# darcamo/pyphysim

Hardware: AMD Instinct MI355X
Metric: Monte Carlo realizations/sec (whole node) + SER abs-error vs ref (higher is better)
Workload: dtype f64

## Files before the change

include/mcle.h:

```cpp
#ifndef MCLE_H
#define MCLE_H

#include <stddef.h>
#include <stdint.h>

#ifdef __cplusplus
extern "C" {
#endif

#define MCLE_VERSION 1

enum { MCLE_OK = 0, MCLE_E_INVAL = -1, MCLE_E_HIP = -2, MCLE_E_NOMEM = -3, MCLE_E_STATE = -4,
       MCLE_E_UNSUPPORTED = -5  };
enum { MCLE_F32 = 0, MCLE_F64 = 1 };
enum { MCLE_DEMOD_MINDIST = 0, MCLE_DEMOD_QAM_SLICER = 1 };
enum { MCLE_CONST_GENERIC = 0, MCLE_CONST_QAM = 1, MCLE_CONST_BPSK = 2 };

typedef struct mcle_ctx mcle_ctx;

typedef struct mcle_counters {
    uint64_t n_realizations;
    uint64_t n_skipped;
    uint64_t sym_errors;
    uint64_t sym_errors_sq;
// ... 10 lines not shown
int mcle_ctx_destroy(mcle_ctx* ctx);
int mcle_ctx_set_stream(mcle_ctx* ctx, void* hip_stream);
int mcle_ctx_get_stream(mcle_ctx* ctx, void** hip_stream);
int mcle_ctx_sync(mcle_ctx* ctx);
int mcle_ctx_trim_scratch(mcle_ctx* ctx);
int mcle_ctx_device_info(mcle_ctx* ctx, int* n_cu, int* lds_bytes, char* name, int name_len);
int mcle_ctx_last_kernel(mcle_ctx* ctx, char* name, int len);
int mcle_malloc(mcle_ctx* ctx, size_t bytes, void** d_ptr);
int mcle_free(mcle_ctx* ctx, void* d_ptr);
int mcle_memset(mcle_ctx* ctx, void* d_ptr, int value, size_t bytes);
int mcle_memcpy_h2d(mcle_ctx* ctx, void* d_dst, const void* src, size_t bytes);
int mcle_memcpy_d2h(mcle_ctx* ctx, void* dst, const void* d_src, size_t bytes);
int mcle_memcpy_2d(mcle_ctx* ctx, void* d_dst, size_t dst_pitch, const void* d_src, size_t src_pitch,
                   size_t row_bytes, size_t rows);
enum {
    MCLE_OPT_NO_MFMA = 0,
    MCLE_OPT_MFMA_VARIANT = 1,
    MCLE_OPT_GRID_OVERSUB = 2,
    MCLE_OPT_FLAT_WGS_PER_CU = 3,
    MCLE_OPT_SINGLE_TDL = 4,
    MCLE_OPT_TDL_MFMA_WAVES = 5,
    MCLE_OPT_JAKES_DIRECT = 6,
    MCLE_OPT_F64_GENERIC = 7,
    MCLE_OPT_F64_THREADS = 8,
    MCLE_OPT_BD_RUNTIME_SOLVE = 9,
    MCLE_OPT_DEMOD_NOCERT = 10,
    MCLE_OPT_F64_VARIANT = 11,
    MCLE_OPT_F32_MFMA = 12,
    MCLE_OPT_TDL_KERNEL = 13,
    MCLE_OPT_MIMO_TDL_KERNEL = 14,
    MCLE_OPT_WALK_LEGACY = 15,
    MCLE_OPT_STAGED_GENERIC = 16,
    MCLE_OPT_CODEBOOK_NO_PACK = 17,
    MCLE_OPT_COUNT = 18
};
int mcle_ctx_set_option(mcle_ctx* ctx, int option, long long value);
int mcle_ctx_get_option(mcle_ctx* ctx, int option, long long* value);

int mcle_timer_start(mcle_ctx* ctx);
int mcle_timer_stop_ms(mcle_ctx* ctx, float* ms);

enum { MCLE_HBM_COPY = 0, MCLE_HBM_READ = 1, MCLE_HBM_TRIAD = 2, MCLE_HBM_WRITE = 3,
       MCLE_HBM_NONTEMPORAL = 4 , MCLE_HBM_UNROLL8 = 8  };
int mcle_hbm_stream_rate(mcle_ctx* ctx, int kind, size_t bytes, int reps, int blocks_per_cu, double* gbps);

int mcle_comm_load(const char* rccl_path);
int mcle_comm_unique_id(void* id_out, size_t bytes);
int mcle_comm_init(mcle_ctx* ctx, const void* unique_id, int rank, int world);
int mcle_comm_destroy(mcle_ctx* ctx);
int mcle_comm_info(mcle_ctx* ctx, int* rank, int* world);
int mcle_counters_allreduce(mcle_ctx* ctx, mcle_counters* d_counters, int n);
int mcle_allreduce_f64(mcle_ctx* ctx, double* d_values, size_t n);


int mcle_set_constellation(mcle_ctx* ctx, const double* re_im, int M, int kind);

int mcle_build_demod_grid(const double* re_im, int M, int* G, double* x0, double* y0, double* h,
                          unsigned long long* cells);

int mcle_modulate(mcle_ctx* ctx, int dtype, const int32_t* d_idx, void* d_out, size_t n);
int mcle_demodulate(mcle_ctx* ctx, int dtype, int method, const void* d_rx, int32_t* d_idx,
                    size_t n);
int mcle_count_errors(mcle_ctx* ctx, const int32_t* d_tx_idx, const int32_t* d_rx_idx,
                      size_t n_per_real, size_t n_real, int bits_per_symbol,
                      mcle_counters* d_counters, uint32_t* d_sym_err, uint32_t* d_bit_err);
int mcle_demod_count(mcle_ctx* ctx, int dtype, int method, const void* d_rx,
                     const int32_t* d_tx_idx, size_t n_per_real, size_t n_real,
// ... 429 lines not shown
```

pyphysim_amd/_lib.py:

```python
import ctypes
import importlib.util
import os
from ctypes import (POINTER, Structure, byref, c_char_p, c_double, c_float, c_int, c_int32, c_longlong, c_size_t,
                    c_uint32, c_uint64, c_void_p)

import numpy as np

MCLE_F32, MCLE_F64 = 0, 1
DEMOD_MINDIST, DEMOD_QAM_SLICER = 0, 1
CONST_GENERIC, CONST_QAM, CONST_BPSK = 0, 1, 2
MAX_TAPS = 24
STREAM_DATA, STREAM_NOISE, STREAM_CHAN, STREAM_PHASE, STREAM_PILOT = 0, 1, 2, 3, 4
OPTIONS = {"no_mfma": 0, "mfma_variant": 1, "grid_oversub": 2, "flat_wgs_per_cu": 3, "single_tdl": 4,
           "tdl_mfma_waves": 5, "jakes_direct": 6, "f64_generic": 7,
           "f64_threads": 8, "bd_runtime_solve": 9, "demod_nocert": 10, "f64_variant": 11, "f32_mfma": 12, "tdl_kernel": 13,
           "mimo_tdl_kernel": 14, "walk_legacy": 15, "staged_generic": 16, "codebook_no_pack": 17}

LIB_DIR = os.path.join(os.path.dirname(os.path.abspath(__file__)), "csrc")
LIB_PATH = os.environ.get("MCLE_LIBRARY") or os.path.join(LIB_DIR, "libmcle.so")


class McleError(RuntimeError):
    """Any failure reported by libmcle (message from mcle_last_error)."""


class McleUnsupported(McleError):
    """A valid request outside a fused kernel's envelope (MCLE_E_UNSUPPORTED): use the staged operators."""


class Counters(Structure):
    _fields_ = [(n, c_uint64) for n in ("n_realizations", "n_skipped", "sym_errors", "sym_errors_sq",
                                        "bit_errors", "bit_errors_sq", "n_symbols", "n_bits")]

    def as_dict(self):
        return {n: int(getattr(self, n)) for n, _ in self._fields_}


COUNTER_FIELDS = [n for n, _ in Counters._fields_]


class AwgnCfg(Structure):
    _fields_ = [("n_symbols", c_int32), ("demod_method", c_int32), ("noise_var", c_double)]


class FlatCfg(Structure):
    _fields_ = [("n_symbols", c_int32), ("demod_method", c_int32), ("noise_var", c_double),
                ("Fd", c_double), ("Ts", c_double), ("L", c_int32), ("rayleigh_iid", c_int32)]


# ... 353 lines not shown
```

pyphysim_amd/csrc/c4_select.hpp:

```cpp
#pragma once
#include <cstdio>
#include "../../include/mcle.h"

namespace mcle {

enum : int { WDEC_GENERIC = 0, WDEC_SLICER = 1, WDEC_QAM_CERT = 2, WDEC_QUAD_CERT = 3, WDEC_AXIS4_CERT = 4 };

enum : int {
    C4_THR_DEFAULT = 0,
    C4_THR_R4_AH4 = 256,
    C4_THR_R16_ALT = 257,
    C4_THR_R16_TABLE = 258,
    C4_THR_R16_FUSED = 259,
    C4_THR_WAVE = 260,
    C4_THR_PLANAR = 261,
    C4_THR_WAVE_ALT = 262,
    C4_THR_PW4 = 263,
    C4_THR_PW4_W2 = 264,
    C4_THR_PW_TIME = 265,
    C4_THR_PW_CLASS = 266,
    C4_THR_PW_PLANES = 267,
    C4_THR_PW_HALVES = 268,
    C4_THR_512 = 512,
    C4_THR_1024 = 1024,
};
constexpr bool c4_threads_accepted(long long v) {
    return v == C4_THR_DEFAULT || (v >= C4_THR_R4_AH4 && v <= C4_THR_PW_HALVES) || v == C4_THR_512 || v == C4_THR_1024;
}

struct C4Query {
    bool f64;
    int fft_size, nt, nr, num_used, cp_size;
    int M;
    int dec;
    long long f64_threads, f64_generic, no_mfma, f32_mfma, mfma_variant;
#ifdef MCLE_EXPERIMENTS
    long long f64_variant;
#endif
};

enum : int { C4_REFUSED_SHAPE = 0, C4_GENERIC, C4_PLANAR, C4_FW, C4_QW, C4_PW, C4_MFMA };

struct C4Plan {
    int family = C4_REFUSED_SHAPE;
    bool f64 = true;
    int n = 0, nt = 0, nr = 0;
    int ah = 0;
    int wps = 0;
    int variant = 0;
    bool td = false, rows = false, halves = false;
    char asked = 0;
    int abl = 0;
};

#ifndef MCLE_PLANAR_F32_WPS_PLUS
#define MCLE_PLANAR_F32_WPS_PLUS 2
#endif
#ifndef MCLE_PLANAR_F64_256_WPS3
#define MCLE_PLANAR_F64_256_WPS3 0
#endif
constexpr int planar_wps(bool f64, int n, int nt, int nr, int w64) {
    if (!f64 && w64 <= 3 && ((n == 256 && !(nt == 4 && nr == 4)) || (n == 512 && nr == 2))) return w64 + MCLE_PLANAR_F32_WPS_PLUS;
    if (MCLE_PLANAR_F64_256_WPS3 && f64 && n == 256 && nr <= 3 && w64 == 2) return 3;
    return w64;
}

constexpr int planar_r4_ah(int nr) { return nr == 3 ? 3 : 2; }
constexpr int planar_r4_wps(bool f64, int n, int nt, int nr) {
    const int w64 = nr == 3 ? 2 : nr == 2 ? (n == 256 ? 2 : n == 2048 ? 4 : 3) : (n <= 512 ? 3 : 4);
    return planar_wps(f64, n, nt, nr, w64);
}

#ifdef MCLE_EXPERIMENTS
constexpr bool c4_abl_wave(long long v) { return (v >= 32 && v <= 1024 && (v & (v - 1)) == 0) || v == 2016; }
constexpr bool c4_abl_qw(long long v) { return c4_abl_wave(v) || v == 384; }
constexpr bool c4_abl_planar(long long v) { return c4_abl_qw(v) || v == 1920; }
#endif

inline bool c4_select_planar(const C4Query& q, C4Plan& p) {
    const int n = q.fft_size, nt = q.nt, nr = q.nr;
    const long long thr = q.f64_threads;
    if (!(n == 256 || n == 512 || n == 1024 || n == 2048) || nr < 2 || nr > 4 || nt < 1 || nt > nr) return false;
    if (n == 256 && nt == 2 && nr == 2) return false;
    p.family = C4_PLANAR;
    p.ah = planar_r4_ah(nr);
    p.wps = planar_r4_wps(q.f64, n, nt, nr);
    p.variant = 0;
    if (n == 1024 && nr == 4) {
        const int r16_wps = q.f64 ? 2 : 4, r16_var = q.f64 ? 12 : 4;
        if (nt < 4) {
            if (thr == C4_THR_DEFAULT) p.ah = 4, p.wps = r16_wps, p.variant = r16_var;
            return true;
        }
#ifdef MCLE_EXPERIMENTS
        if (q.f64 && q.f64_variant >= 1 && q.f64_variant <= 3) {
            p.variant = (int)q.f64_variant;
            return true;
        }
        if (q.f64 && c4_abl_planar(q.f64_variant)) {
            p.ah = 4, p.wps = 2, p.variant = 12 | (int)q.f64_variant;
            return true;
        }
#endif
        if (thr == C4_THR_512) return true;
// ... 12 lines not shown
inline C4Plan c4_select(const C4Query& q) {
    const int n = q.fft_size, nt = q.nt, nr = q.nr;
    const long long thr = q.f64_threads;
    const bool sq4 = nt == 4 && nr == 4;
    C4Plan p;
    p.f64 = q.f64, p.n = n, p.nt = nt, p.nr = nr;
    if (!q.f64 && q.f32_mfma && !q.no_mfma && n == 1024 && sq4) {
        p.family = C4_MFMA;
        p.variant = q.mfma_variant ? (int)q.mfma_variant : 36;
        return p;
    }
    const bool has_generic = nt == nr && (nt == 2 || nt == 4);
    const bool want_generic = has_generic && (q.f64_generic || (!q.f64 && q.no_mfma));
    if (!want_generic) {
        const bool wave = q.num_used == n && (q.cp_size & 1) == 0 && q.M <= 256 && q.dec != WDEC_GENERIC;
        const bool wave_thr = thr == C4_THR_DEFAULT || thr == C4_THR_WAVE || thr == C4_THR_WAVE_ALT;
        if (wave && n == 256 && has_generic && wave_thr) {
            p.family = C4_FW;
            p.wps = (thr == C4_THR_WAVE_ALT) == q.f64 ? 2 : 3;
#ifdef MCLE_EXPERIMENTS
            if (q.f64 && sq4 && c4_abl_wave(q.f64_variant)) p.wps = 3, p.abl = (int)q.f64_variant;
#endif
            return p;
        }
        const bool pw_thr = thr == C4_THR_DEFAULT || (thr >= C4_THR_PW_TIME && thr <= C4_THR_PW_HALVES) ||
                            (n == 1024 ? thr == C4_THR_PW4 || thr == C4_THR_PW4_W2 : thr == C4_THR_WAVE || thr == C4_THR_WAVE_ALT);
        if (wave && q.f64 && sq4 && (n == 512 || n == 1024 || n == 2048) && pw_thr) {
            p.family = C4_PW;
            p.wps = n == 2048 ? 2 : 3;
            p.td = thr == C4_THR_PW_TIME;
            p.rows = !p.td && thr != C4_THR_PW_CLASS;
            p.halves = p.rows && (thr == C4_THR_PW_HALVES || (thr != C4_THR_PW_PLANES && n != 512));
            p.asked = thr == C4_THR_PW_PLANES ? 'x' : thr == C4_THR_PW_HALVES ? 'h' : 0;
            if (n != 2048) {
                if (thr == C4_THR_WAVE_ALT || thr == C4_THR_PW4_W2) p.wps = 2;
#ifdef MCLE_EXPERIMENTS
                if ((thr < C4_THR_PW_CLASS || thr > C4_THR_PW_HALVES) && c4_abl_wave(q.f64_variant))
                    p.wps = 3, p.halves = false, p.abl = (int)q.f64_variant;
#endif
            }
            return p;
        }
        if (wave && q.f64 && sq4 && n == 1024 && wave_thr && (q.dec == WDEC_SLICER || q.dec == WDEC_QAM_CERT || q.dec == WDEC_QUAD_CERT)) {
            p.family = C4_QW;
            p.wps = thr == C4_THR_WAVE_ALT ? 2 : 3;
#ifdef MCLE_EXPERIMENTS
            if (c4_abl_qw(q.f64_variant)) p.wps = 3, p.abl = (int)q.f64_variant;
#endif
            return p;
        }
        if (c4_select_planar(q, p)) return p;
    }
    if (has_generic) p.family = C4_GENERIC;
    return p;
}

inline void c4_plan_tag(const C4Plan& p, char* out, int len) {
    const char* dt = p.f64 ? "f64" : "f32";
    switch (p.family) {
        case C4_GENERIC: std::snprintf(out, (size_t)len, "mimo_ofdm_generic<%d,%d> %s", p.n, p.nt, dt); break;
        case C4_PLANAR: std::snprintf(out, (size_t)len, "mimo_ofdm_planar<%d,%d,%d> %s ah%d w%d v%d", p.n, p.nt, p.nr, dt, p.ah, p.wps, p.variant); break;
        case C4_FW: std::snprintf(out, (size_t)len, "mimo_ofdm_fw<%d> %s w%d", p.nt, dt, p.wps); break;
        case C4_QW: std::snprintf(out, (size_t)len, "mimo_ofdm_qw w%d", p.wps); break;
        case C4_PW:
            std::snprintf(out, (size_t)len, "mimo_ofdm_pw<%d>/%s%s%s", p.n / 256, p.td ? "time" : "freq", p.wps == (p.n == 2048 ? 2 : 3) ? "" : "/w2",
                          !p.td && !p.rows ? "/a" : p.asked == 'x' ? "/x" : p.asked == 'h' ? "/h" : "");
// ... 8 lines not shown
```

pyphysim_amd/csrc/capi.hip:

```cpp
#include <cmath>
#include <cstdarg>

#include "c4_select.hpp"
#include "common.hpp"
#include "modem.hpp"

namespace mcle {

static thread_local char g_err[512] = "";

void set_error(const char* fmt, ...) {
    va_list ap;
    va_start(ap, fmt);
    vsnprintf(g_err, sizeof(g_err), fmt, ap);
    va_end(ap);
}

}

using namespace mcle;

int mcle_ctx::bind() const {
    MCLE_HIP(hipSetDevice(device));
    return MCLE_OK;
// ... 177 lines not shown
}

int mcle_ctx_get_stream(mcle_ctx* ctx, void** hip_stream) {
    MCLE_REQUIRE(ctx != nullptr && hip_stream != nullptr, "null argument");
    *hip_stream = (void*)ctx->stream;
    return MCLE_OK;
}

int mcle_ctx_set_option(mcle_ctx* ctx, int option, long long value) {
    MCLE_REQUIRE(ctx != nullptr, "null context");
    MCLE_REQUIRE(option >= 0 && option < MCLE_OPT_COUNT, "unknown option %d", option);
    bool ok = false;
    switch (option) {
        case MCLE_OPT_NO_MFMA: case MCLE_OPT_SINGLE_TDL: case MCLE_OPT_JAKES_DIRECT: case MCLE_OPT_F64_GENERIC: case MCLE_OPT_BD_RUNTIME_SOLVE: case MCLE_OPT_DEMOD_NOCERT: case MCLE_OPT_F32_MFMA: case MCLE_OPT_WALK_LEGACY: case MCLE_OPT_STAGED_GENERIC: case MCLE_OPT_CODEBOOK_NO_PACK: ok = value == 0 || value == 1; break;
        case MCLE_OPT_TDL_KERNEL: ok = value >= 0 && value <= 4; break;
#ifdef MCLE_EXPERIMENTS
        case MCLE_OPT_MIMO_TDL_KERNEL: ok = value >= 0 && value <= 255; break;
#else
        case MCLE_OPT_MIMO_TDL_KERNEL: ok = value >= 0 && value <= 2; break;
#endif
#ifdef MCLE_EXPERIMENTS
        case MCLE_OPT_F64_VARIANT: ok = value >= 0 && value <= 2047; break;
#else
        case MCLE_OPT_F64_VARIANT:
            MCLE_REQUIRE(value == 0, "option MCLE_OPT_F64_VARIANT: the timing-bound variants are compiled with -DMCLE_EXPERIMENTS only");
            ok = true;
            break;
#endif
        case MCLE_OPT_MFMA_VARIANT: ok = value == 0 || value == 36 || value == 32 || value == 30 || value == 21; break;
        case MCLE_OPT_GRID_OVERSUB: ok = value >= 0 && value <= 64; break;
        case MCLE_OPT_FLAT_WGS_PER_CU: ok = value >= 0 && value <= 4096; break;
        case MCLE_OPT_TDL_MFMA_WAVES: ok = value == 0 || value == 2 || value == 3 || value == 32; break;
        case MCLE_OPT_F64_THREADS: ok = c4_threads_accepted(value); break;
    }
    MCLE_REQUIRE(ok, "option %d: value %lld out of range", option, value);
    ctx->opt[option] = value;
    return MCLE_OK;
}

int mcle_ctx_trim_scratch(mcle_ctx* ctx) {
    MCLE_REQUIRE(ctx != nullptr, "null context");
    MCLE_HIP(hipSetDevice(ctx->device));
    MCLE_HIP(hipStreamSynchronize(ctx->stream));
    if (ctx->d_scratch) MCLE_HIP(hipFree(ctx->d_scratch));
    ctx->d_scratch = nullptr;
    ctx->scratch_bytes = 0;
    return MCLE_OK;
}

int mcle_ctx_get_option(mcle_ctx* ctx, int option, long long* value) {
    MCLE_REQUIRE(ctx != nullptr && value != nullptr, "null argument");
    MCLE_REQUIRE(option >= 0 && option < MCLE_OPT_COUNT, "unknown option %d", option);
    *value = ctx->opt[option];
    return MCLE_OK;
}

int mcle_ctx_sync(mcle_ctx* ctx) {
    MCLE_REQUIRE(ctx != nullptr, "null context");
    MCLE_HIP(hipSetDevice(ctx->device));
    MCLE_HIP(hipStreamSynchronize(ctx->stream));
    return MCLE_OK;
}

int mcle_ctx_device_info(mcle_ctx* ctx, int* n_cu, int* lds_bytes, char* name, int name_len) {
    MCLE_REQUIRE(ctx != nullptr, "null context");
    if (n_cu) *n_cu = ctx->n_cu;
// ... 303 lines not shown
```

pyphysim_amd/csrc/pipeline_mimo_pw.hip:

```cpp
#include "mimo_planar_common.hpp"
#include "walk_f64.hpp"

namespace mcle {

constexpr int kPwPlane = 4 * 272;
__host__ __device__ __forceinline__ int pw_slot(int a, int e) { return a * 272 + e + (e >> 4); }
__host__ __device__ __forceinline__ int pw_mtime(int h, int c) { return (c & 3) * 64 + (c >> 2) * 16 + (h & 3) * 4 + (h >> 2); }
template <int NW> constexpr int pw_lab_stride() { return 16 * NW + 16; }
template <int NW> constexpr size_t pw_static_lds() {
    return (size_t)((kBmLdsDoubles + 1) & ~1) * sizeof(double) + (size_t)64 * pw_lab_stride<NW>() + 2 * (d64_rec<4, 4>() + 1) * sizeof(double2) +
           64 * sizeof(unsigned) + sizeof(WgTotals);
}

__device__ __forceinline__ void pw_row_swap(uint32_t& x, uint32_t& y) {
#if defined(__HIP_DEVICE_COMPILE__)
#if __has_builtin(__builtin_amdgcn_permlane16_swap)
    const auto s = __builtin_amdgcn_permlane16_swap(x, y, false, false);
    x = s[0];
    y = s[1];
#else
    const bool odd = (__lane_id() & 16) != 0;
    const uint32_t give = odd ? x : y, got = (uint32_t)__shfl_xor((int)give, 16);
    if (odd) x = got;
    else y = got;
#endif
#endif
}

template <int NW, int J, bool STUB>
__device__ __forceinline__ void pw_first_stage(const unsigned char* lab_row, const double2* s_txtab, const double2* __restrict__ g_tw,
                                               double2 (&v)[16]) {
    const uint4* lab = reinterpret_cast<const uint4*>(lab_row);
    if constexpr (NW == 4) {
#pragma unroll
        for (int i = 0; i < 4; ++i) {
            const uint4 L = lab[i];
            const uint32_t wds[4] = {L.x, L.y, L.z, L.w};
#pragma unroll
            for (int uu = 0; uu < 4; ++uu) {
                const int u = 4 * i + uu;
                const uint32_t w = wds[uu];
                double2 X0, X1, X2, X3;
                if constexpr (STUB) {
                    X0 = X1 = X2 = X3 = mk<double>((double)w, 1.0);
// ... 60 lines not shown
                else v[u] = cmulc(S, g_tw[16 * J * u]);
            }
        }
    } else {
        static_assert(NW == 2, "first stage");
#pragma unroll
        for (int i = 0; i < 2; ++i) {
            const uint4 L = lab[i];
            const uint32_t wds[4] = {L.x, L.y, L.z, L.w};
#pragma unroll
            for (int uu = 0; uu < 8; ++uu) {
                const int u = 8 * i + uu;
                const uint32_t w = wds[uu >> 1] >> (16 * (uu & 1));
                double2 X0, X1;
                if constexpr (STUB) {
                    X0 = X1 = mk<double>((double)(w & 0xFFFFu), 1.0);
                } else {
                    X0 = s_txtab[w & 0xFFu];
                    X1 = s_txtab[(w >> 8) & 0xFFu];
                }
                const double2 S = J ? csub(X0, X1) : cadd(X0, X1);
                if constexpr (J == 0) v[u] = S;
                else if (u == 0) v[u] = S;
                else v[u] = cmulc(S, g_tw[16 * J * u]);
            }
        }
    }
}

template <int NW, int DEC, int WPS, bool TD = false, int ABL = 0, bool ROWS = !TD, bool XCH = ROWS && !TD>
__global__ __launch_bounds__(64 * NW, WPS) void k_run_mimo_ofdm_pw(MimoParams pp, ModemParams<double> mp, uint64_t seed, uint64_t first,
                                                                   uint64_t count, const double2* __restrict__ g_tw,
                                                                   const double2* __restrict__ g_recs, mcle_counters* counters,
                                                                   uint32_t* __restrict__ sym_out, uint32_t* __restrict__ bit_out) {
    using T = double;
    constexpr int N = 256 * NW, NT = 4, NR = 4, kRec = d64_rec<NT, NR>(), TB = 64 * NW, UU = 16 / NW;
    constexpr int kLabStride = pw_lab_stride<NW>();
    static_assert(NW == 2 || NW == 4 || NW == 8, "wavefronts per realization");
    static_assert(!(TD && ROWS), "the time-domain form keeps the map wavefront = class");
    static_assert(!XCH || (ROWS && ABL == 0), "the exchange in complex halves belongs to the default form by lane row");
    constexpr bool kAhead = ROWS && ABL == 0;
#ifdef MCLE_PW_LATE_B5
    constexpr bool kLateB5 = XCH && kAhead;
#else
    constexpr bool kLateB5 = false;
#endif
    constexpr int kLogNW = NW == 2 ? 1 : NW == 4 ? 2 : 3;
    extern __shared__ __attribute__((aligned(16))) char pw_smem[];
    constexpr int kBm = (kBmLdsDoubles + 1) & ~1;
    __shared__ __attribute__((aligned(16))) double s_bm[kBm];
    __shared__ __attribute__((aligned(16))) unsigned char s_lab[64 * kLabStride];
    __shared__ __attribute__((aligned(16))) cx<T> s_rec[2 * (kRec + 1)];
    __shared__ unsigned s_part[64];
    __shared__ WgTotals totals;
    static_assert(sizeof(s_bm) + sizeof(s_lab) + sizeof(s_rec) + sizeof(s_part) + sizeof(totals) == pw_static_lds<NW>(), "launcher's LDS sum");
    T* s_R = reinterpret_cast<T*>(pw_smem);
    cx<T>* s_table = reinterpret_cast<cx<T>*>(s_R + NW * kPwPlane);
    cx<T>* s_txtab = s_table + ((mp.M + 1) & ~1);

    const int tid = threadIdx.x, lane = tid & 63;
    const int j = __builtin_amdgcn_readfirstlane(tid >> 6);
    const int pj = j & 1;
    const int cp = pp.cp;
    const int per_sym = N * NT;
    const uint64_t row = (uint64_t)pp.n_ofdm_sym * (N + cp);
    const T sigma = (T)sqrt(pp.noise_var);
    const T tx_scale = (T)(1.0 / sqrt((double)NT) / sqrt((double)(N + cp)));
    const T tab_scale = TD ? tx_scale : tx_scale * (T)N;
    const uint32_t mask = (uint32_t)(mp.M - 1);
    for (int m = tid; m < mp.M; m += TB) {
        const cx<T> c = mp.g_table[m];
        s_table[m] = c;
        s_txtab[m] = cscale(c, tab_scale);
    }
    if constexpr (ROWS) bm_tables_to_lds_pairs(s_bm, tid, TB);
    else bm_tables_to_lds(s_bm, tid, TB);
    if (tid == 0) wg_zero(totals);

    T* s_mine = s_R + j * kPwPlane;
    uint2* s_words_mine = reinterpret_cast<uint2*>(s_mine);
    using Pass = std::conditional_t<kAhead, uint32_t, uint64_t>;
    Pass it = 0;
    uint64_t rl_prev = 0;
    cx<T> rec_next = mk<T>(0, 0);
    if (tid < kRec && blockIdx.x < count) rec_next = g_recs[(uint64_t)blockIdx.x * kRec + tid];
    unsigned step = 0;
    if constexpr (kAhead) {
        step = gridDim.x;
        asm volatile("" : "+s"(step));
    }
    auto grid_step = [&]() -> unsigned {
        if constexpr (kAhead) return step;
        else return gridDim.x;
    };
    __syncthreads();
    for (uint64_t rl = blockIdx.x; rl < count; rl += grid_step(), ++it) {
        const Rng rng(seed, first + rl);
        const int buf = (int)(it & 1);
        if (tid < kRec) {
            s_rec[buf * (kRec + 1) + tid] = rec_next;
            if (rl + grid_step() < count) rec_next = g_recs[(rl + grid_step()) * kRec + tid];
        }
        const cx<T>* s_H = s_rec + buf * (kRec + 1);
        const cx<T>* s_G = s_H + NT * NR;
        unsigned se = 0, be = 0;
        for (int os = 0; os < pp.n_ofdm_sym; ++os) {
            if constexpr (!kLateB5) {
                if (it > 0 || os > 0) __syncthreads();
            }
            if constexpr (ROWS && !(ABL & 128)) __builtin_amdgcn_s_waitcnt(0xC07F);
            {
                const int t = opaque(tid);
                Words4 dw;
                if constexpr (ABL & 32) dw.w[0] = dw.w[1] = dw.w[2] = dw.w[3] = (uint32_t)t * 0x01010101u;
                else dw = rng.block(STREAM_DATA, (uint32_t)(((uint64_t)os * per_sym) >> 4) + (uint32_t)t);
                const int q = (t >> 6) ^ (NW / 2), u = (t & 63) >> 2;
#pragma unroll
                for (int s = 0; s < 4; ++s) {
                    const uint32_t w = dw.w[s] & (mask * 0x01010101u);
                    const int g = 4 * (t & 3) + s;
                    unsigned char* dst = s_lab + g * kLabStride + NW * u + q;
#pragma unroll
                    for (int a = 0; a < 4; ++a) dst[a * 16 * kLabStride] = (unsigned char)(w >> (8 * a));
                }
            }
            if constexpr (!ROWS) {
                const int ln = opaque(lane);
                const int r = ln >> 4, h = ln & 15;
                const uint64_t i00 = (uint64_t)r * row + (uint64_t)os * (N + cp) + cp + (j & ~1) + 32 * NW * pj + NW * (uint64_t)pw_mtime(h, 0);
                const uint32_t b0 = (uint32_t)(i00 >> 1);
                uint2* w_even = reinterpret_cast<uint2*>(s_R + (j & ~1) * kPwPlane) + (8 * pj) * 64 + ln;
                uint2* w_odd = reinterpret_cast<uint2*>(s_R + (j | 1) * kPwPlane) + (8 * pj) * 64 + ln;
#pragma unroll
                for (int cc = 0; cc < 8; ++cc) {
                    Words4 b;
                    if constexpr (ABL & 128) b.w[0] = b.w[1] = b.w[2] = b.w[3] = b0 + cc;
                    else b = rng.block(STREAM_NOISE, b0 + (uint32_t)(NW / 2) * (uint32_t)pw_mtime(0, cc));
                    w_even[cc * 64] = make_uint2(b.w[0], b.w[1]);
                    w_odd[cc * 64] = make_uint2(b.w[2], b.w[3]);
                }
            }
            auto account_prev = [&]() {
                if (tid == 0 && os == 0 && it > 0) {
                    const unsigned* qq = s_part + (buf ^ 1) * 32;
                    unsigned ts = 0, tb = 0;
#pragma unroll
                    for (int i = 0; i < NW; ++i) {
                        ts += qq[2 * i];
                        tb += qq[2 * i + 1];
                    }
                    uint64_t rp = rl_prev;
                    if constexpr (kAhead) {
                        uint64_t here = rl;
                        asm volatile("" : "+s"(here));
                        rp = here - step;
                    }
                    wg_account(totals, ts, tb, s_rec[(buf ^ 1) * (kRec + 1) + 2 * NT * NR].x != 0.0, rp, sym_out, bit_out);
                }
            };
            if constexpr (!ROWS) {
                __syncthreads();
                account_prev();
            }
            cx<T> v[16];
            if constexpr (TD) {
                const int ln = opaque(lane);
                const unsigned char* lab = s_lab + ln * kLabStride;
                if constexpr (NW == 4) {
                    switch (j) {
                        case 0: pw_first_stage<4, 0, (ABL & 32) != 0>(lab, s_txtab, g_tw, v); break;
                        case 1: pw_first_stage<4, 1, (ABL & 32) != 0>(lab, s_txtab, g_tw, v); break;
                        case 2: pw_first_stage<4, 2, (ABL & 32) != 0>(lab, s_txtab, g_tw, v); break;
                        default: pw_first_stage<4, 3, (ABL & 32) != 0>(lab, s_txtab, g_tw, v); break;
                    }
                } else if constexpr (NW == 8) {
                    switch (j) {
                        case 0: pw_first_stage<8, 0, (ABL & 32) != 0>(lab, s_txtab, g_tw, v); break;
                        case 1: pw_first_stage<8, 1, (ABL & 32) != 0>(lab, s_txtab, g_tw, v); break;
                        case 2: pw_first_stage<8, 2, (ABL & 32) != 0>(lab, s_txtab, g_tw, v); break;
                        case 3: pw_first_stage<8, 3, (ABL & 32) != 0>(lab, s_txtab, g_tw, v); break;
                        case 4: pw_first_stage<8, 4, (ABL & 32) != 0>(lab, s_txtab, g_tw, v); break;
                        case 5: pw_first_stage<8, 5, (ABL & 32) != 0>(lab, s_txtab, g_tw, v); break;
                        case 6: pw_first_stage<8, 6, (ABL & 32) != 0>(lab, s_txtab, g_tw, v); break;
                        default: pw_first_stage<8, 7, (ABL & 32) != 0>(lab, s_txtab, g_tw, v); break;
                    }
                } else {
                    if (j == 0) pw_first_stage<2, 0, (ABL & 32) != 0>(lab, s_txtab, g_tw, v);
                    else pw_first_stage<2, 1, (ABL & 32) != 0>(lab, s_txtab, g_tw, v);
// ... 349 lines not shown
                    T keep = er[0][0] + ei[NW - 1][UU - 1];
                    if constexpr (!TD) {
#pragma unroll
                        for (int u = 0; u < 16; ++u) keep += v[u].x + v[u].y;
                    }
                    se += (unsigned)(keep == 0.5) + (wds[0] == 0x12345u);
                }
            }
        }
        if constexpr (kAhead) {
            se = walk_wave_total(se);
            be = walk_wave_total(be);
        } else {
            se = wave_sum_u32(se);
            be = wave_sum_u32(be);
        }
        if (lane == 0) {
            s_part[buf * 32 + 2 * j] = se;
            s_part[buf * 32 + 2 * j + 1] = be;
        }
        rl_prev = rl;
    }
    __syncthreads();
    if (tid == 0) {
        if (it > 0) {
            const int buf = (int)((it - 1) & 1);
            const unsigned* qq = s_part + buf * 32;
            unsigned ts = 0, tb = 0;
#pragma unroll
            for (int i = 0; i < NW; ++i) {
                ts += qq[2 * i];
                tb += qq[2 * i + 1];
            }
            if constexpr (kAhead) rl_prev = blockIdx.x + (uint64_t)(it - 1) * step;
            wg_account(totals, ts, tb, s_rec[buf * (kRec + 1) + 2 * NT * NR].x != 0.0, rl_prev, sym_out, bit_out);
        }
        wg_flush(totals, counters, (unsigned long long)per_sym * pp.n_ofdm_sym, (unsigned long long)per_sym * pp.n_ofdm_sym * mp.bits);
    }
}

template <int NW, int WPS, bool TD, int ABL, bool ROWS, bool XCH>
static int launch_mimo_ofdm_pw(mcle_ctx* ctx, const C4Plan& plan, const mcle_mimo_ofdm_cfg* cfg, uint64_t seed, uint64_t first,
                               uint64_t count, mcle_counters* d_counters, uint32_t* d_sym, uint32_t* d_bit) {
    using T = double;
    constexpr int N = 256 * NW, NT = 4, NR = 4;
    int rc;
    void* tw = nullptr;
    if ((rc = ctx->get_twiddles(N, MCLE_F64, &tw))) return rc;
    MimoParams pp{cfg->cp_size, cfg->num_used, cfg->n_ofdm_sym, cfg->mmse, cfg->noise_var};
    ModemParams<T> mp = pipe_modem<T>(ctx, cfg->demod_method);
    const int dec = walk_dec_kind(ctx, mp);
    mp.grid.G = 0;
    const size_t tab_len = ((size_t)mp.M + 1) & ~(size_t)1;
    const size_t dyn = (size_t)NW * kPwPlane * sizeof(T) + 2 * tab_len * sizeof(cx<T>);
    const size_t lds = dyn + pw_static_lds<NW>();
    MCLE_REQUIRE(lds + 512 <= (size_t)160 * 1024, "part-wave MIMO-OFDM kernel: %zu B of LDS do not fit", lds);
    auto kern = k_run_mimo_ofdm_pw<NW, WDEC_SLICER, WPS, TD, ABL, ROWS, XCH>;
    switch (dec) {
        case WDEC_QAM_CERT: kern = k_run_mimo_ofdm_pw<NW, WDEC_QAM_CERT, WPS, TD, ABL, ROWS, XCH>; break;
        case WDEC_QUAD_CERT: kern = k_run_mimo_ofdm_pw<NW, WDEC_QUAD_CERT, WPS, TD, ABL, ROWS, XCH>; break;
        case WDEC_AXIS4_CERT: kern = k_run_mimo_ofdm_pw<NW, WDEC_AXIS4_CERT, WPS, TD, ABL, ROWS, XCH>; break;
        default: break;
    }
    MCLE_HIP(hipFuncSetAttribute((const void*)kern, hipFuncAttributeMaxDynamicSharedMemorySize, (int)dyn));
    int per_cu = (int)((size_t)160 * 1024 / (lds + 512));
    if (per_cu < 1) per_cu = 1;
    const int by_waves = WPS * 4 / NW;
    if (per_cu > by_waves) per_cu = by_waves;
    const uint64_t resident = (uint64_t)ctx->n_cu * per_cu;
    static_assert(XCH ? ROWS && ABL == 0 : true, "the exchange in complex halves: default form by lane row only");
    set_c4_kernel(ctx, plan);
    const uint64_t kSlice = 1ull << 20;
    return launch_sliced_planar<T, N, NT, NR>(ctx, pp, seed, first, count, kSlice, d_sym, d_bit,
                                              [&](void* recs, uint64_t at, uint64_t n, uint32_t* sym, uint32_t* bit) {
        const unsigned grid = (unsigned)oversubscribed_grid(ctx, resident, n, 8, NW == 4 ? 32 : 16);
        hipLaunchKernelGGL(kern, dim3(grid), dim3(64 * NW), dyn, ctx->stream, pp, mp, seed, at, n, (const cx<T>*)tw, (const cx<T>*)recs,
                           d_counters, sym, bit);
    });
}

int launch_mimo_ofdm_pw(mcle_ctx* ctx, const C4Plan& p, const mcle_mimo_ofdm_cfg* cfg, uint64_t seed, uint64_t first, uint64_t count,
                        mcle_counters* d_counters, uint32_t* d_sym, uint32_t* d_bit) {
#define MCLE_PW(NW_, WPS_, TD_, ABL_, ROWS_, XCH_)                                                                              \
    if (p.n == 256 * NW_ && p.wps == WPS_ && p.td == TD_ && p.abl == ABL_ && p.rows == ROWS_ && p.halves == XCH_)               \
        return launch_mimo_ofdm_pw<NW_, WPS_, TD_, ABL_, ROWS_, XCH_>(ctx, p, cfg, seed, first, count, d_counters, d_sym, d_bit);
#define MCLE_PW_SIZE(NW_, WPS_)                                                                                                 \
    MCLE_PW(NW_, WPS_, false, 0, false, false) MCLE_PW(NW_, WPS_, false, 0, true, true) MCLE_PW(NW_, WPS_, false, 0, true, false) \
    MCLE_PW(NW_, WPS_, true, 0, false, false)
    MCLE_PW_SIZE(2, 3) MCLE_PW(2, 2, false, 0, true, false)
    MCLE_PW_SIZE(4, 3) MCLE_PW(4, 2, false, 0, true, true)
    MCLE_PW_SIZE(8, 2)
#ifdef MCLE_EXPERIMENTS
#define MCLE_PW_ABL(V_)                                                                                                         \
    MCLE_PW(2, 3, true, V_, false, false) MCLE_PW(2, 3, false, V_, true, false) MCLE_PW(4, 3, true, V_, false, false)           \
    MCLE_PW(4, 3, false, V_, true, false)
    MCLE_PW_ABL(32) MCLE_PW_ABL(64) MCLE_PW_ABL(128) MCLE_PW_ABL(256) MCLE_PW_ABL(512) MCLE_PW_ABL(1024) MCLE_PW_ABL(2016)
#undef MCLE_PW_ABL
#endif
#undef MCLE_PW_SIZE
#undef MCLE_PW
    MCLE_REQUIRE(false, "internal: no part-wave MIMO-OFDM kernel <%d> w%d time %d rows %d halves %d ablation %d", p.n / 256, p.wps, (int)p.td,
                 (int)p.rows, (int)p.halves, p.abl);
}

}
```

pyphysim_amd/csrc/pipelines.hip:

```cpp
#include <cstdlib>

#include "fft.hpp"
#include "jakes.hpp"
#include "mimo.hpp"
#include "modem.hpp"
#include "philox.hpp"
#include "totals.hpp"
#include "pipe_common.hpp"
#include "qam_pack.hpp"
#include "walk_f64.hpp"

namespace mcle {


__global__ __launch_bounds__(256) void k_fold_counters(const unsigned* __restrict__ ws,
                                                       const unsigned* __restrict__ skipped, size_t n_real,
                                                       unsigned long long n_sym, unsigned long long n_bits,
                                                       mcle_counters* counters, uint32_t* __restrict__ sym_out,
                                                       uint32_t* __restrict__ bit_out) {
    unsigned long long se = 0, se2 = 0, be = 0, be2 = 0, ok = 0, sk = 0;
    for (size_t r = (size_t)blockIdx.x * blockDim.x + threadIdx.x; r < n_real; r += (size_t)gridDim.x * blockDim.x) {
        const bool skip = skipped && skipped[r];
        const unsigned long long s = ws[2 * r], t = ws[2 * r + 1];
        if (sym_out) sym_out[r] = skip ? 0xFFFFFFFFu : (uint32_t)s;
// ... 1018 lines not shown
    }
    fp.noise_sigma = std::sqrt(cfg->noise_var);
    if (dtype == MCLE_F32)
        return run_flat_impl<float>(ctx, fp, cfg->demod_method, seed, first, count, d_counters, d_sym_err, d_bit_err);
    return run_flat_impl<double>(ctx, fp, cfg->demod_method, seed, first, count, d_counters, d_sym_err, d_bit_err);
}

int mcle_run_mimo_ofdm(mcle_ctx* ctx, int dtype, const mcle_mimo_ofdm_cfg* cfg, uint64_t seed, uint64_t first,
                       uint64_t count, mcle_counters* d_counters, uint32_t* d_sym_err, uint32_t* d_bit_err) {
    if (ctx) ctx->last_kernel[0] = 0;
    int rc = check_pipe(ctx, dtype, cfg ? cfg->demod_method : 0, cfg);
    if (rc) return rc;
    MCLE_REQUIRE(cfg->nt >= 1 && cfg->nt <= cfg->nr && cfg->nr <= 4, "fused MIMO pipeline: 1 <= Nt <= Nr <= 4 (got %d x %d)",
                 cfg->nt, cfg->nr);
    MCLE_REQUIRE(cfg->cp_size >= 0 && cfg->cp_size <= cfg->fft_size,
                 "cp_size must be nonnegative and cannot be greater than fft_size");
    MCLE_REQUIRE(cfg->num_used >= 2 && cfg->num_used % 2 == 0 && cfg->num_used <= cfg->fft_size,
                 "Number of used subcarriers must be a multiple of 2 and at most fft_size");
    MCLE_REQUIRE(cfg->n_ofdm_sym >= 1, "n_ofdm_sym must be positive");
    MCLE_REQUIRE(cfg->noise_var >= 0.0, "Noise variance must be a non-negative value.");
    MCLE_REQUIRE(count <= 0x7fffffffull, "at most 2^31-1 realizations per call");
    if (count == 0) return MCLE_OK;
    if ((rc = ctx->bind())) return rc;
    C4Query q{};
    q.f64 = dtype == MCLE_F64;
    q.fft_size = cfg->fft_size, q.nt = cfg->nt, q.nr = cfg->nr, q.num_used = cfg->num_used, q.cp_size = cfg->cp_size;
    q.M = ctx->M;
    {
        ModemParams<double> mp = pipe_modem<double>(ctx, cfg->demod_method);
        q.dec = walk_dec_kind(ctx, mp);
    }
    q.f64_threads = ctx->opt[MCLE_OPT_F64_THREADS], q.f64_generic = ctx->opt[MCLE_OPT_F64_GENERIC];
    q.no_mfma = ctx->opt[MCLE_OPT_NO_MFMA], q.f32_mfma = ctx->opt[MCLE_OPT_F32_MFMA], q.mfma_variant = ctx->opt[MCLE_OPT_MFMA_VARIANT];
#ifdef MCLE_EXPERIMENTS
    q.f64_variant = ctx->opt[MCLE_OPT_F64_VARIANT];
#endif
    const C4Plan plan = c4_select(q);
    switch (plan.family) {
        case C4_MFMA: return launch_mimo_ofdm_mfma(ctx, plan, cfg, seed, first, count, d_counters, d_sym_err, d_bit_err);
        case C4_PLANAR: return launch_mimo_ofdm_planar(ctx, plan, cfg, seed, first, count, d_counters, d_sym_err, d_bit_err);
        case C4_FW: return launch_mimo_ofdm_fw(ctx, plan, cfg, seed, first, count, d_counters, d_sym_err, d_bit_err);
        case C4_QW: return launch_mimo_ofdm_qw(ctx, plan, cfg, seed, first, count, d_counters, d_sym_err, d_bit_err);
        case C4_PW: return launch_mimo_ofdm_pw(ctx, plan, cfg, seed, first, count, d_counters, d_sym_err, d_bit_err);
        case C4_GENERIC: break;
        default:
            MCLE_REQUIRE(false, "fused MIMO pipeline: %d x %d at fft_size %d is outside the envelope (2x2 / 4x4 at 64 .. 2048 in both arithmetics; "
                         "every 1 <= Nt <= Nr <= 4 with Nr >= 2 at 256 .. 2048)", cfg->nt, cfg->nr, cfg->fft_size);
    }
#define MCLE_RUN(N_, NA_)                                                                                               \
    if (plan.n == N_ && plan.nt == NA_)                                                                                 \
        return plan.f64 ? run_mimo_impl<double, N_, NA_>(ctx, plan, cfg, seed, first, count, d_counters, d_sym_err, d_bit_err) \
                        : run_mimo_impl<float, N_, NA_>(ctx, plan, cfg, seed, first, count, d_counters, d_sym_err, d_bit_err);
    MCLE_RUN(64, 2) MCLE_RUN(64, 4) MCLE_RUN(128, 2) MCLE_RUN(128, 4) MCLE_RUN(256, 2) MCLE_RUN(256, 4)
    MCLE_RUN(512, 2) MCLE_RUN(512, 4) MCLE_RUN(1024, 2) MCLE_RUN(1024, 4) MCLE_RUN(2048, 2) MCLE_RUN(2048, 4)
#undef MCLE_RUN
    set_error("fused MIMO pipeline supports fft_size in {64, 128, ..., 2048} (got %d)", cfg->fft_size);
    return MCLE_E_INVAL;
}

int mcle_run_ofdm_tdl(mcle_ctx* ctx, int dtype, const mcle_ofdm_tdl_cfg* cfg, uint64_t seed, uint64_t first,
                      uint64_t count, mcle_counters* d_counters, uint32_t* d_sym_err, uint32_t* d_bit_err) {
    if (ctx) ctx->last_kernel[0] = 0;
    int rc = check_pipe(ctx, dtype, cfg ? cfg->demod_method : 0, cfg);
    if (rc) return rc;
    MCLE_REQUIRE(cfg->cp_size >= 0 && cfg->cp_size <= cfg->fft_size,
                 "cp_size must be nonnegative and cannot be greater than fft_size");
// ... 33 lines not shown
```

Measured before the change: 50.19 million.

## Replace grid-stride loop in PW MIMO kernel with guided contiguous chunk schedule

Replaces the grid-stride realization loop in the PW MIMO-OFDM kernel with a host-computed schedule. Workgroups get contiguous ranges of realizations in rounds of geometrically shrinking chunks (ratio 1/2, floor 8 by default), which should balance tail work and give contiguous record prefetch. It adds a new option to pick the ratio and floor or fall back to a uniform oversubscription, and passes the schedule struct as a kernel argument. Risks are more workgroups, extra per-block index arithmetic, and uneven tail behaviour if the chunk sizing is off.

```diff
diff --git a/include/mcle.h b/include/mcle.h
--- a/include/mcle.h
+++ b/include/mcle.h
@@ -66,7 +66,8 @@
     MCLE_OPT_WALK_LEGACY = 15,
     MCLE_OPT_STAGED_GENERIC = 16,
     MCLE_OPT_CODEBOOK_NO_PACK = 17,
-    MCLE_OPT_COUNT = 18
+    MCLE_OPT_PW_SCHEDULE = 18,
+    MCLE_OPT_COUNT = 19
 };
 int mcle_ctx_set_option(mcle_ctx* ctx, int option, long long value);
 int mcle_ctx_get_option(mcle_ctx* ctx, int option, long long* value);
diff --git a/pyphysim_amd/_lib.py b/pyphysim_amd/_lib.py
--- a/pyphysim_amd/_lib.py
+++ b/pyphysim_amd/_lib.py
@@ -14,7 +14,8 @@
 OPTIONS = {"no_mfma": 0, "mfma_variant": 1, "grid_oversub": 2, "flat_wgs_per_cu": 3, "single_tdl": 4,
            "tdl_mfma_waves": 5, "jakes_direct": 6, "f64_generic": 7,
            "f64_threads": 8, "bd_runtime_solve": 9, "demod_nocert": 10, "f64_variant": 11, "f32_mfma": 12, "tdl_kernel": 13,
-           "mimo_tdl_kernel": 14, "walk_legacy": 15, "staged_generic": 16, "codebook_no_pack": 17}
+           "mimo_tdl_kernel": 14, "walk_legacy": 15, "staged_generic": 16, "codebook_no_pack": 17,
+           "pw_schedule": 18}
 
 LIB_DIR = os.path.join(os.path.dirname(os.path.abspath(__file__)), "csrc")
 LIB_PATH = os.environ.get("MCLE_LIBRARY") or os.path.join(LIB_DIR, "libmcle.so")
diff --git a/pyphysim_amd/csrc/c4_schedule.hpp b/pyphysim_amd/csrc/c4_schedule.hpp
--- /dev/null
+++ b/pyphysim_amd/csrc/c4_schedule.hpp
@@ -0,0 +1,77 @@
+#pragma once
+#include <cstdint>
+
+namespace mcle {
+
+constexpr int kPwMaxRounds = 16;
+constexpr uint64_t kPwMaxOversub = 32;
+
+struct PwSchedule {
+    uint32_t n_wg;
+    uint32_t rounds;
+    uint32_t last_wg0;
+    uint32_t extra;
+    uint32_t wg0[kPwMaxRounds];
+    struct Round {
+        uint32_t base;
+        uint32_t chunk;
+    } round[kPwMaxRounds];
+};
+
+constexpr uint64_t pw_uniform_f(uint64_t count, uint64_t resident, uint64_t min_units, uint64_t max_f) {
+    uint64_t f = max_f;
+    while (f > 1 && count < resident * f * min_units) f >>= 1;
+    return f;
+}
+
+inline PwSchedule pw_schedule(uint64_t count, uint64_t resident, uint64_t min_chunk, uint64_t num, uint64_t den, uint64_t forced_f) {
+    PwSchedule s{};
+    for (int r = 0; r < kPwMaxRounds; ++r) s.wg0[r] = 0xffffffffu;
+    if (count == 0) return s;
+    if (resident < 1) resident = 1;
+    if (min_chunk < 1) min_chunk = 1;
+    if (forced_f > kPwMaxOversub) forced_f = kPwMaxOversub;
+    auto one_round = [&](uint64_t want) {
+        const uint64_t g = count < want ? count : want;
+        for (int r = 1; r < kPwMaxRounds; ++r) s.wg0[r] = 0xffffffffu, s.round[r].base = 0, s.round[r].chunk = 0;
+        s.n_wg = (uint32_t)g, s.rounds = 1, s.last_wg0 = 0, s.extra = (uint32_t)(count % g);
+        s.wg0[0] = 0, s.round[0].base = 0, s.round[0].chunk = (uint32_t)(count / g);
+    };
+    if (forced_f > 0) {
+        one_round(resident * forced_f);
+        return s;
+    }
+    if (num == 0 || den == 0 || count < resident * min_chunk) {
+        one_round(resident);
+        return s;
+    }
+    uint64_t rem = count, at = 0, wg = 0, prev = ~0ull;
+    int r = 0;
+    while (r < kPwMaxRounds - 1 && rem > 0) {
+        uint64_t c = rem * num / den / resident;
+        if (c > prev) c = prev;
+        if (c < min_chunk) break;
+        s.wg0[r] = (uint32_t)wg, s.round[r].base = (uint32_t)at, s.round[r].chunk = (uint32_t)c;
+        wg += resident, at += resident * c, rem -= resident * c, prev = c;
+        ++r;
+    }
+    if (rem > 0) {
+        uint64_t n = (rem + min_chunk - 1) / min_chunk;
+        const uint64_t fill = rem < resident ? rem : resident;
+        if (n < fill) n = fill;
+        s.wg0[r] = (uint32_t)wg, s.round[r].base = (uint32_t)at, s.round[r].chunk = (uint32_t)(rem / n);
+        s.extra = (uint32_t)(rem % n);
+        wg += n;
+        ++r;
+    }
+    s.rounds = (uint32_t)r, s.last_wg0 = s.wg0[r - 1], s.n_wg = (uint32_t)wg;
+    if (wg > resident * kPwMaxOversub) one_round(resident * kPwMaxOversub);
+    return s;
+}
+
+constexpr bool pw_schedule_accepted(long long v) { return v == 0 || v == 1 || (v >= 256 + 1 && v <= 3 * 256 + 64 && (v & 255) >= 1 && (v & 255) <= 64); }
+constexpr long long pw_schedule_value(int ratio, int floor) { return 256ll * ratio + floor; }
+constexpr uint64_t pw_ratio_num(int ratio) { return ratio == 1 ? 1 : ratio == 2 ? 2 : ratio == 3 ? 3 : 0; }
+constexpr uint64_t pw_ratio_den(int ratio) { return ratio == 1 ? 2 : ratio == 2 ? 3 : 4; }
+
+}
diff --git a/pyphysim_amd/csrc/c4_select.hpp b/pyphysim_amd/csrc/c4_select.hpp
--- a/pyphysim_amd/csrc/c4_select.hpp
+++ b/pyphysim_amd/csrc/c4_select.hpp
@@ -1,6 +1,7 @@
 #pragma once
 #include <cstdio>
 #include "../../include/mcle.h"
+#include "c4_schedule.hpp"
 
 namespace mcle {
 
@@ -34,6 +35,7 @@
     int M;
     int dec;
     long long f64_threads, f64_generic, no_mfma, f32_mfma, mfma_variant;
+    long long pw_schedule;
 #ifdef MCLE_EXPERIMENTS
     long long f64_variant;
 #endif
@@ -50,6 +52,7 @@
     int variant = 0;
     bool td = false, rows = false, halves = false;
     char asked = 0;
+    int pw_sched = 1;
     int abl = 0;
 };
 
@@ -70,6 +73,8 @@
     const int w64 = nr == 3 ? 2 : nr == 2 ? (n == 256 ? 2 : n == 2048 ? 4 : 3) : (n <= 512 ? 3 : 4);
     return planar_wps(f64, n, nt, nr, w64);
 }
+
+constexpr int pw_sched_default(int ) { return (int)pw_schedule_value(1, 8); }
 
 #ifdef MCLE_EXPERIMENTS
 constexpr bool c4_abl_wave(long long v) { return (v >= 32 && v <= 1024 && (v & (v - 1)) == 0) || v == 2016; }
@@ -148,6 +153,7 @@
             p.rows = !p.td && thr != C4_THR_PW_CLASS;
             p.halves = p.rows && (thr == C4_THR_PW_HALVES || (thr != C4_THR_PW_PLANES && n != 512));
             p.asked = thr == C4_THR_PW_PLANES ? 'x' : thr == C4_THR_PW_HALVES ? 'h' : 0;
+            p.pw_sched = q.pw_schedule ? (int)q.pw_schedule : pw_sched_default(n);
             if (n != 2048) {
                 if (thr == C4_THR_WAVE_ALT || thr == C4_THR_PW4_W2) p.wps = 2;
 #ifdef MCLE_EXPERIMENTS
diff --git a/pyphysim_amd/csrc/capi.hip b/pyphysim_amd/csrc/capi.hip
--- a/pyphysim_amd/csrc/capi.hip
+++ b/pyphysim_amd/csrc/capi.hip
@@ -233,6 +233,7 @@
         case MCLE_OPT_FLAT_WGS_PER_CU: ok = value >= 0 && value <= 4096; break;
         case MCLE_OPT_TDL_MFMA_WAVES: ok = value == 0 || value == 2 || value == 3 || value == 32; break;
         case MCLE_OPT_F64_THREADS: ok = c4_threads_accepted(value); break;
+        case MCLE_OPT_PW_SCHEDULE: ok = pw_schedule_accepted(value); break;
     }
     MCLE_REQUIRE(ok, "option %d: value %lld out of range", option, value);
     ctx->opt[option] = value;
diff --git a/pyphysim_amd/csrc/pipeline_mimo_pw.hip b/pyphysim_amd/csrc/pipeline_mimo_pw.hip
--- a/pyphysim_amd/csrc/pipeline_mimo_pw.hip
+++ b/pyphysim_amd/csrc/pipeline_mimo_pw.hip
@@ -10,6 +10,23 @@
 template <int NW> constexpr size_t pw_static_lds() {
     return (size_t)((kBmLdsDoubles + 1) & ~1) * sizeof(double) + (size_t)64 * pw_lab_stride<NW>() + 2 * (d64_rec<4, 4>() + 1) * sizeof(double2) +
            64 * sizeof(unsigned) + sizeof(WgTotals);
+}
+
+__device__ __forceinline__ void pw_share(const PwSchedule& s, uint64_t count, uint32_t& lo, uint32_t& hi) {
+    const uint32_t b = blockIdx.x;
+    int r = -1;
+#pragma unroll
+    for (int i = 0; i < kPwMaxRounds; ++i) r += b >= s.wg0[i] ? 1 : 0;
+    r = r < 0 ? 0 : r;
+    const uint32_t w0 = s.wg0[r], ba = s.round[r].base, ch = s.round[r].chunk;
+    const uint32_t k = b - w0;
+    const uint32_t ex = w0 == s.last_wg0 ? s.extra : 0u;
+    uint64_t l = (uint64_t)ba + (uint64_t)k * ch + (k < ex ? k : ex);
+    uint64_t h = l + ch + (k < ex ? 1u : 0u);
+    h = h < count ? h : count;
+    l = l < h ? l : h;
+    lo = (uint32_t)__builtin_amdgcn_readfirstlane((int)(uint32_t)l);
+    hi = (uint32_t)__builtin_amdgcn_readfirstlane((int)(uint32_t)h);
 }
 
 __device__ __forceinline__ void pw_row_swap(uint32_t& x, uint32_t& y) {
@@ -136,7 +153,8 @@
 __global__ __launch_bounds__(64 * NW, WPS) void k_run_mimo_ofdm_pw(MimoParams pp, ModemParams<double> mp, uint64_t seed, uint64_t first,
                                                                    uint64_t count, const double2* __restrict__ g_tw,
                                                                    const double2* __restrict__ g_recs, mcle_counters* counters,
-                                                                   uint32_t* __restrict__ sym_out, uint32_t* __restrict__ bit_out) {
+                                                                   uint32_t* __restrict__ sym_out, uint32_t* __restrict__ bit_out,
+                                                                   PwSchedule sch) {
     using T = double;
     constexpr int N = 256 * NW, NT = 4, NR = 4, kRec = d64_rec<NT, NR>(), TB = 64 * NW, UU = 16 / NW;
     constexpr int kLabStride = pw_lab_stride<NW>();
@@ -187,23 +205,16 @@
     Pass it = 0;
     uint64_t rl_prev = 0;
     cx<T> rec_next = mk<T>(0, 0);
-    if (tid < kRec && blockIdx.x < count) rec_next = g_recs[(uint64_t)blockIdx.x * kRec + tid];
-    unsigned step = 0;
-    if constexpr (kAhead) {
-        step = gridDim.x;
-        asm volatile("" : "+s"(step));
-    }
-    auto grid_step = [&]() -> unsigned {
-        if constexpr (kAhead) return step;
-        else return gridDim.x;
-    };
+    uint32_t lo, hi;
+    pw_share(sch, count, lo, hi);
+    if (tid < kRec && lo < hi) rec_next = g_recs[(uint64_t)lo * kRec + tid];
     __syncthreads();
-    for (uint64_t rl = blockIdx.x; rl < count; rl += grid_step(), ++it) {
+    for (uint64_t rl = lo; rl < hi; ++rl, ++it) {
         const Rng rng(seed, first + rl);
         const int buf = (int)(it & 1);
         if (tid < kRec) {
             s_rec[buf * (kRec + 1) + tid] = rec_next;
-            if (rl + grid_step() < count) rec_next = g_recs[(rl + grid_step()) * kRec + tid];
+            if (rl + 1 < hi) rec_next = g_recs[(rl + 1) * kRec + tid];
         }
         const cx<T>* s_H = s_rec + buf * (kRec + 1);
         const cx<T>* s_G = s_H + NT * NR;
@@ -257,7 +268,7 @@
                     if constexpr (kAhead) {
                         uint64_t here = rl;
                         asm volatile("" : "+s"(here));
-                        rp = here - step;
+                        rp = here - 1;
                     }
                     wg_account(totals, ts, tb, s_rec[(buf ^ 1) * (kRec + 1) + 2 * NT * NR].x != 0.0, rp, sym_out, bit_out);
                 }
@@ -673,7 +684,7 @@
                 ts += qq[2 * i];
                 tb += qq[2 * i + 1];
             }
-            if constexpr (kAhead) rl_prev = blockIdx.x + (uint64_t)(it - 1) * step;
+            if constexpr (kAhead) rl_prev = (uint64_t)hi - 1;
             wg_account(totals, ts, tb, s_rec[buf * (kRec + 1) + 2 * NT * NR].x != 0.0, rl_prev, sym_out, bit_out);
         }
         wg_flush(totals, counters, (unsigned long long)per_sym * pp.n_ofdm_sym, (unsigned long long)per_sym * pp.n_ofdm_sym * mp.bits);
@@ -714,9 +725,12 @@
     const uint64_t kSlice = 1ull << 20;
     return launch_sliced_planar<T, N, NT, NR>(ctx, pp, seed, first, count, kSlice, d_sym, d_bit,
                                               [&](void* recs, uint64_t at, uint64_t n, uint32_t* sym, uint32_t* bit) {
-        const unsigned grid = (unsigned)oversubscribed_grid(ctx, resident, n, 8, NW == 4 ? 32 : 16);
-        hipLaunchKernelGGL(kern, dim3(grid), dim3(64 * NW), dyn, ctx->stream, pp, mp, seed, at, n, (const cx<T>*)tw, (const cx<T>*)recs,
-                           d_counters, sym, bit);
+        const int ratio = plan.pw_sched >> 8, floor = plan.pw_sched & 255;
+        uint64_t forced = ctx->opt[MCLE_OPT_GRID_OVERSUB] > 0 ? (uint64_t)ctx->opt[MCLE_OPT_GRID_OVERSUB] : 0;
+        if (forced == 0 && ratio == 0) forced = pw_uniform_f(n, resident, 8, NW == 4 ? 32 : 16);
+        const PwSchedule sch = pw_schedule(n, resident, (uint64_t)floor, pw_ratio_num(ratio), pw_ratio_den(ratio), forced);
+        hipLaunchKernelGGL(kern, dim3(sch.n_wg), dim3(64 * NW), dyn, ctx->stream, pp, mp, seed, at, n, (const cx<T>*)tw, (const cx<T>*)recs,
+                           d_counters, sym, bit, sch);
     });
 }
 
diff --git a/pyphysim_amd/csrc/pipelines.hip b/pyphysim_amd/csrc/pipelines.hip
--- a/pyphysim_amd/csrc/pipelines.hip
+++ b/pyphysim_amd/csrc/pipelines.hip
@@ -1074,6 +1074,7 @@
     }
     q.f64_threads = ctx->opt[MCLE_OPT_F64_THREADS], q.f64_generic = ctx->opt[MCLE_OPT_F64_GENERIC];
     q.no_mfma = ctx->opt[MCLE_OPT_NO_MFMA], q.f32_mfma = ctx->opt[MCLE_OPT_F32_MFMA], q.mfma_variant = ctx->opt[MCLE_OPT_MFMA_VARIANT];
+    q.pw_schedule = ctx->opt[MCLE_OPT_PW_SCHEDULE];
 #ifdef MCLE_EXPERIMENTS
     q.f64_variant = ctx->opt[MCLE_OPT_F64_VARIANT];
 #endif
```

After: 50.36 million, median of 6. About the same (+0.3%).
